# UT-Austin-RPL/GIGA

Measured on AMD Instinct MI355X. Metric: scenes/sec, higher is better.
Workload: dtype f32

## Files before the change

giga_amd/csrc/giga_encoder.hip:

```cpp
#include <atomic>
#include <cstdlib>

#include "../../include/giga_hip.h"
#include "giga_dev.h"
#include "giga_conv16.h"
#include "giga_conv32.h"
#include "giga_wino.h"
#include "giga_bwd_mega.h"
#include "giga_args.h"

namespace giga {



constexpr int CV_RS = 44;
constexpr int CV_OFF = 3;
constexpr int CV_ROWS = 12;
constexpr int ci_red_units(int nw) { return nw == 4 ? 25 : 13; }
constexpr size_t ci_lds_bytes(int xw, int nw, bool f16class = false) {
    const size_t stage = ((size_t)(xw + 3) * (f16class ? CI16_SLAB : CV_ROWS * CV_RS) + 4) * sizeof(float);
    const size_t red = (size_t)nw * ci_red_units(nw) * 64 * 16;
    return stage > red ? stage : red;
}

#ifdef GIGA_TRACE
static __device__ long long g_ci_trace[8 * 64];
#define CI_T(idx) do { if (blockIdx.x == 43 && lane == 0) \
        g_ci_trace[wave * 64 + (idx)] = __builtin_amdgcn_s_memtime(); } while (0)
#else
#define CI_T(idx) do {} while (0)
#endif
template <typename TOut, int SXW, bool SPLIT = false, int NW = 8, bool LO = true, bool MASK = false>
__global__ __launch_bounds__(512) void convin_project_kernel(
    const float* __restrict__ tsdf,
    const float* __restrict__ wpk,
    const float* __restrict__ bias,
    TOut* __restrict__ planes,
    float* __restrict__ xz_partial,
    float* __restrict__ yz_partial,
    int B, uint4* __restrict__ relu_mask = nullptr) {
    constexpr int XW = NW * SXW, NT = NW * 64;
    constexpr bool F16C = SPLIT || sizeof(TOut) == 2;
    constexpr int RS = SPLIT ? CI16_RS : CV_RS, SLAB = SPLIT ? CI16_SLAB : CV_ROWS * CV_RS;
    extern __shared__ __attribute__((aligned(16))) float lds[];
    const int tid = threadIdx.x, lane = tid & 63;
    const int wave = __builtin_amdgcn_readfirstlane(tid >> 6);
    const int j = lane & 15, g = lane >> 4;
    int xp = blockIdx.x, wy = blockIdx.y, b = blockIdx.z;
    if constexpr (XW == RES) {
        const int i = blockIdx.x, nfull = (B >> 3) << 6;
        xp = 0;
        if (i < nfull) { const int xcd = i & 7, slot = i >> 3; b = (slot >> 3) * 8 + xcd; wy = slot & 7; }
        else           { b = i >> 3; wy = i & 7; }
    }
    const int grp = wy >> 1, chh = wy & 1;
    const int x0 = xp * XW;
    const float* vol = tsdf + (size_t)b * RES * RES * RES;
    CI_T(0);

    constexpr int SPP = NT / 120, NPASS = (XW + 2 + SPP - 1) / SPP;
    const int st_slab = tid / 120, st_e = tid - 120 * st_slab, st_yl = st_e / 10, st_q = st_e - 10 * st_yl;
    const int st_iy = 10 * grp - 1 + st_yl;
    const bool st_on = st_slab < SPP && st_iy >= 0 && st_iy < RES;
    const float* st_src = vol + ((size_t)(x0 - 1 + st_slab) * RES + st_iy) * RES + 4 * st_q;
    float4 vals[NPASS];
#pragma unroll
    for (int p = 0; p < NPASS; ++p) {
        const int xl = st_slab + SPP * p, ix = x0 - 1 + xl;
        vals[p] = make_float4(0.f, 0.f, 0.f, 0.f);
        if (st_on && xl < XW + 2 && ix >= 0 && ix < RES)
            vals[p] = *reinterpret_cast<const float4*>(st_src + (size_t)SPP * p * RES * RES);
    }
    CI_T(50);
    float wreg[7];
    half8 wsh = {0, 0, 0, 0, 0, 0, 0, 0}, wsl = wsh;
    if constexpr (SPLIT) {
        const half8* wsp = reinterpret_cast<const half8*>(wpk);
        wsh = wsp[(2 * chh) * 64 + lane];
        wsl = wsp[(2 * chh + 1) * 64 + lane];
    } else {
#pragma unroll
        for (int s = 0; s < 7; ++s) wreg[s] = wpk[(chh * 7 + s) * 64 + lane];
    }
    const int ch = 16 * chh + j;
    const float bn = bias[ch];
    int abase[7];
#pragma unroll
    for (int s = 0; s < 7; ++s) {
        int t = 4 * s + g;
        t = t > 26 ? 26 : t;
        abase[s] = (t / 9) * SLAB + ((j >> 3) + (t / 3) % 3) * RS + CV_OFF + 4 * ((j >> 2) & 1) + (j & 3) + t % 3;
    }
    int sbase[8];
#pragma unroll
    for (int e = 0; e < 8; ++e) {
        const int t = g == 0 ? ci16_read(0, e) : g == 1 ? ci16_read(1, e) : g == 2 ? ci16_read(2, e) : ci16_read(3, e);
        sbase[e] = (t / 9) * SLAB + ((j >> 3) + (t / 3) % 3) * RS + CV_OFF + 4 * ((j >> 2) & 1) + (j & 3) + t % 3;
    }
    f32x4v acc_yz[5][5];
#pragma unroll
    for (int ip = 0; ip < 5; ++ip)
#pragma unroll
        for (int zg = 0; zg < 5; ++zg) acc_yz[ip][zg] = f32x4v{0.f, 0.f, 0.f, 0.f};
    const float inv = 1.0f / RES;
    const size_t img_stride = (size_t)RES * RES * CD;
    TOut* plane_xy = planes + ((size_t)1 * B + b) * img_stride;
    TOut* plane_yz = planes + ((size_t)2 * B + b) * img_stride;
    float* xzp = xz_partial + ((size_t)grp * B + b) * img_stride;
    const f32x4v bias4 = {bn, bn, bn, bn};
    const f32x4v zero4 = {0.f, 0.f, 0.f, 0.f};
    const unsigned xz_lane_b = ((4 * (g & 1) + 2 * (g >> 1)) * RES * CD + ch) * 4u;
    auto xz_store = [&](const f32x4v& part, float* dst) {
        float a02 = part[0], b02 = part[2], a13 = part[1], b13 = part[3];
        lane32_swap(a02, b02);
        lane32_swap(a13, b13);
        store_f32_saddr(dst, xz_lane_b, a02 + b02);
        store_f32_saddr(dst + RES * CD, xz_lane_b, a13 + b13);
    };
    auto xy_store = [&](const f32x2v (&sz)[5], TOut* dst) {
#pragma unroll
        for (int ia = 0; ia < 5; ia += 2) {
            const int ib = ia + 1 < 5 ? ia + 1 : ia;
            float sa = sz[ia][0] + sz[ia][1], sb = sz[ib][0] + sz[ib][1];
            lane16_swap(sa, sb);
            if (ia != ib || (g & 1) == 0) {
                const int iy = grp * 10 + 2 * (ia + (g & 1) * (ib - ia)) + (g >> 1);
                dst[iy * RES * CD + ch] = (TOut)((sa + sb) * inv);
            }
        }
    };
    if (st_slab < SPP) {
        float* st_dst = lds + st_slab * SLAB + st_yl * RS + CV_OFF + 1 + 4 * st_q;
#pragma unroll
        for (int p = 0; p < NPASS; ++p) {
            if (st_slab + SPP * p >= XW + 2) break;
            float* dst = st_dst + SPP * p * SLAB;
            float4 val = vals[p];
            if constexpr (SPLIT) {
                float* v4 = reinterpret_cast<float*>(&val);
#pragma unroll
// ... 167 lines not shown
            const int u = u0 + ul, ip = u / 5, zg = u % 5, lg = ln >> 4, lj = ln & 15;
            const int iy = grp * 10 + 2 * ip + (lg >> 1), iz0 = 8 * zg + 4 * (lg & 1);
            const int di = (iz0 * RES + iy) * CD + 16 * chh + lj;
            if constexpr (XW == RES) {
#pragma unroll
                for (int r = 0; r < 4; ++r) plane_yz[di + r * RES * CD] = (TOut)(sum[r] * inv);
            } else {
#pragma unroll
                for (int r = 0; r < 4; ++r) yzp[di + r * RES * CD] = sum[r];
            }
        }
        CI_T(41 + rd);
    }
    CI_T(63);
}

template <typename TOut>
__global__ void plane_finalize_kernel(const float* __restrict__ xz_partial, const float* __restrict__ yz_partial,
                                      TOut* __restrict__ planes, int B, int nxp, unsigned* __restrict__ sync_words, int nsync) {
    const size_t per4 = (size_t)B * RES * RES * CD / 4;
    const size_t t = (size_t)blockIdx.x * blockDim.x + threadIdx.x;
    if (blockIdx.x == 0 && sync_words) for (int i = threadIdx.x; i < nsync; i += blockDim.x) sync_words[i] = 0u;
    if (t >= per4) return;
    const f32x4v* xs = reinterpret_cast<const f32x4v*>(xz_partial) + t;
    const f32x4v* ys = reinterpret_cast<const f32x4v*>(yz_partial) + t;
    typedef TOut out4 __attribute__((ext_vector_type(4)));
    f32x4v sx = (xs[0] + xs[per4]) + (xs[2 * per4] + xs[3 * per4]);
    out4 ox;
#pragma unroll
    for (int r = 0; r < 4; ++r) ox[r] = (TOut)(sx[r] * (1.0f / RES));
    *reinterpret_cast<out4*>(planes + 4 * t) = ox;
    if (nxp > 1) {
        f32x4v sy = ys[0];
        for (int k = 1; k < nxp; ++k) sy += ys[(size_t)k * per4];
        out4 oy;
#pragma unroll
        for (int r = 0; r < 4; ++r) oy[r] = (TOut)(sy[r] * (1.0f / RES));
        *reinterpret_cast<out4*>(planes + 2 * 4 * per4 + 4 * t) = oy;
    }
}

int enc_nxp(int B) { return B >= 32 ? 1 : 5; }

EncWs enc_workspace(int B, int precision) {
    const size_t es = precision == 1 ? 2 : 4;
    const size_t n = 3 * (size_t)B;
    EncWs w{};
    size_t at = 0;
    auto take = [&](size_t elems, size_t esz) { size_t o = at; at += align_up(elems * esz, 256); return o; };
    w.P0 = take(n * 1600 * 32, es); w.A0 = take(n * 1600 * 32, es); w.S0 = take(n * 1600 * 32, es);
    w.Q0 = take(n * 400 * 32, es);  w.A1 = take(n * 400 * 64, es);  w.S1 = take(n * 400 * 64, es);
    w.Q1 = take(n * 100 * 64, es);  w.A2 = take(n * 100 * 128, es); w.S2 = take(n * 100 * 128, es);
    w.U0 = take(n * 400 * 64, es);  w.A3 = take(n * 400 * 64, es);  w.A4 = take(n * 400 * 64, es);
    w.U1 = take(n * 1600 * 32, es); w.A5 = take(n * 1600 * 32, es); w.A6 = take(n * 1600 * 32, es);
    w.YZ = take((size_t)(4 + enc_nxp(B)) * B * 1600 * 32, 4);
    w.XZ = w.YZ;
    w.SYNC = take(MEGA_SYNC_WORDS * 4, 4);
    w.MASK = take((size_t)B * 8 * RES * 64 * 4, 4);
    w.total = at;
    return w;
}


#define GIGA_UNET_LAYERS(X)                              \
    X(0, CONV3, 32, 0, 32, 40, 40, 2, false, 2)          \
    X(1, CONV3, 32, 0, 32, 40, 40, 2, true, 2)           \
    X(2, CONV3, 32, 0, 64, 20, 20, 1, false, 4)          \
    X(3, CONV3, 64, 0, 64, 20, 20, 1, true, 4)           \
    X(4, CONV3, 64, 0, 128, 10, 10, 1, false, 4)         \
    X(5, CONV3, 128, 0, 128, 10, 10, 1, false, 2)        \
    X(6, UPCONV, 128, 0, 64, 10, 10, 2, false, 2)        \
    X(7, CONV3, 64, 64, 64, 20, 20, 1, false, 2)         \
    X(8, CONV3, 64, 0, 64, 20, 20, 1, false, 4)          \
    X(9, UPCONV, 64, 0, 32, 20, 20, 2, false, 2)         \
    X(10, CONV3, 32, 32, 32, 40, 40, 2, false, 2)        \
    X(11, CONV3, 32, 0, 32, 40, 40, 2, false, 2)         \
    X(12, CONV1, 32, 0, 32, 40, 40, 2, false, 2)

struct MegaArgs {
    ConvArgs layer[NCONV];
    unsigned* sync;
    int nlayers;
    unsigned wino_mask;
};
constexpr int MEGA_GROUP = 8;
constexpr int MEGA_SLOTS = 4;
constexpr int MEGA_GROUP_MAX_IMG = 32;
constexpr int MEGA_NW = CONV_NW;
constexpr unsigned long long MEGA_SPIN_TICKS = 20ull * 100000000ull;
constexpr int MEGA_MAX_IN_FLIGHT = 4;

template <typename T, int MATH, bool WINO = false>
constexpr size_t mega_lds_bytes() {
    size_t m = 0;
#define X(l, KIND, C0, C1, COUT, H, W, NB, POOL, NB16) \
    { constexpr size_t v = conv_lds_bytes<T, KIND, C0, C1, COUT, H, W, (sizeof(T) == 2 ? NB16 : NB), MATH, (WINO ? WINO_NW : CONV_NW)>(); m = v > m ? v : m; \
      if constexpr (WINO && KIND == CONV3) { constexpr size_t u = wino_lds_bytes<C0, C1, H, W>(); m = u > m ? u : m; } }
    GIGA_UNET_LAYERS(X)
#undef X
    return m;
}

#ifdef GIGA_TRACE
static __device__ long long g_mega_trace[8][32];
#endif
__device__ __forceinline__ void xcd_barrier(unsigned* counter, unsigned target, int idx, int trace_row) {
#ifdef GIGA_TRACE
    if (threadIdx.x == 0 && trace_row >= 0 && trace_row < 8 && idx < 16) g_mega_trace[trace_row][2 * idx] = __builtin_amdgcn_s_memtime();
#endif
    if (threadIdx.x == 0) {
        __hip_atomic_fetch_add(counter, 1u, __ATOMIC_RELAXED, __HIP_MEMORY_SCOPE_WORKGROUP);
        unsigned spins = 0;
        unsigned long long t0 = 0;
        while (__hip_atomic_load(counter, __ATOMIC_RELAXED, __HIP_MEMORY_SCOPE_AGENT) < target) {
            __builtin_amdgcn_s_sleep(1);
            if ((++spins & 1023u) == 0) {
                const unsigned long long now = __builtin_amdgcn_s_memrealtime();
                if (t0 == 0) t0 = now;
                else if (now - t0 > MEGA_SPIN_TICKS) __builtin_trap();
            }
        }
    }
    __syncthreads();
#ifdef GIGA_TRACE
    if (threadIdx.x == 0 && trace_row >= 0 && trace_row < 8 && idx < 16) g_mega_trace[trace_row][2 * idx + 1] = __builtin_amdgcn_s_memtime();
#endif
}

__device__ __forceinline__ void xcd_arrive(unsigned* counter) {
    if (threadIdx.x == 0) __hip_atomic_fetch_add(counter, 1u, __ATOMIC_RELAXED, __HIP_MEMORY_SCOPE_WORKGROUP);
}
__device__ __forceinline__ void xcd_wait(unsigned* counter, unsigned target) {
    if (threadIdx.x == 0) {
        unsigned spins = 0;
        unsigned long long t0 = 0;
        while (__hip_atomic_load(counter, __ATOMIC_RELAXED, __HIP_MEMORY_SCOPE_AGENT) < target) {
            __builtin_amdgcn_s_sleep(1);
            if ((++spins & 1023u) == 0) {
                const unsigned long long now = __builtin_amdgcn_s_memrealtime();
                if (t0 == 0) t0 = now;
                else if (now - t0 > MEGA_SPIN_TICKS) __builtin_trap();
            }
        }
    }
    __syncthreads();
}

template <typename T, int KIND, int C0, int C1, int COUT, int H, int W>
__device__ __forceinline__ ConvArgs conv_image_range(ConvArgs a, int img0, int n) {
    constexpr int IH = KIND == DOWN ? 2 * H : H, IW = KIND == DOWN ? 2 * W : W;
    constexpr int OH = KIND == UPCONV ? 2 * H : H, OW = KIND == UPCONV ? 2 * W : W;
    const size_t s0 = (size_t)IH * IW * (a.cs0 ? a.cs0 : C0), s1 = (size_t)IH * IW * (a.cs1 ? a.cs1 : C1);
    a.in0 = reinterpret_cast<const T*>(a.in0) + img0 * s0;
    if (a.in1) a.in1 = reinterpret_cast<const T*>(a.in1) + img0 * s1;
    a.out = reinterpret_cast<T*>(a.out) + (size_t)img0 * OH * OW * COUT;
    if (a.out_pool) a.out_pool = reinterpret_cast<T*>(a.out_pool) + (size_t)img0 * (H / 2) * (W / 2) * COUT;
    if (a.out_nchw) a.out_nchw += (size_t)img0 * COUT * H * W;
    if (a.mask) a.mask += (size_t)img0 * OH * OW * COUT;
    a.nimg = n;
    if (img0 != 0) a.trace_id = -2;
    return a;
}

template <typename T, int MATH, bool WINO = false>
__global__ __launch_bounds__((WINO ? WINO_NW : MEGA_NW) * 64) void unet_mega_kernel(MegaArgs m) {
    extern __shared__ __attribute__((aligned(16))) uint8_t smem[];
    __shared__ unsigned s_place[2];
    if (threadIdx.x == 0) {
        const unsigned xcc = (unsigned)(__builtin_amdgcn_s_getreg((4 - 1) << 11 | 0 << 6 | 20) & 7);
        s_place[0] = xcc;
        s_place[1] = __hip_atomic_fetch_add(m.sync + xcc * 32, 1u, __ATOMIC_RELAXED, __HIP_MEMORY_SCOPE_WORKGROUP);
    }
    __syncthreads();
    const int xcd = (int)s_place[0], ticket = (int)s_place[1];
    const int nq = (int)gridDim.x >> 3, slot = ticket / MEGA_GROUP, q = slot * 8 + xcd, nimg = m.layer[0].nimg;
    if (slot >= nq >> 3) return;
    const int img0 = (q * nimg + nq - 1) / nq, per = ((q + 1) * nimg + nq - 1) / nq - img0;
    if (per == 0) return;
    const int block = ticket - slot * MEGA_GROUP, nblocks = MEGA_GROUP;
    unsigned* counter = m.sync + (8 + q) * 32;
    unsigned epoch = 0;
    auto is_wino = [&](auto kind_tag, int l) { return WINO && decltype(kind_tag)::value == CONV3 && (m.wino_mask >> l & 1u); };
#define X(l, KIND, C0, C1, COUT, H, W, NB, POOL, NB16)                                                                     \
    if (l < m.nlayers) {                                                                                                   \
        const ConvArgs a = conv_image_range<T, KIND, C0, C1, COUT, H, W>(m.layer[l], img0, per);                           \
        bool direct = true;                                                                                                \
        if constexpr (WINO && KIND == CONV3) {                                                                             \
            if (is_wino(std::integral_constant<int, KIND>{}, l)) {                                                         \
                direct = false;                                                                                            \
                _Pragma("unroll") for (int k = 0; k < wino_kpass(C0 + C1); ++k) {                                          \
                    if (l == 0 || k > 0) wino_fill<C0, C1, COUT>(a, smem, block, nblocks, k);                              \
                    wino_run<C0, C1, COUT, H, W, POOL, true>(a, smem, block, nblocks, k);                                  \
                    __builtin_amdgcn_s_waitcnt(0x0F70);                                                                    \
                    __syncthreads();                                                                                       \
                }                                                                                                          \
            }                                                                                                              \
        }                                                                                                                  \
        if constexpr (WINO && KIND == UPCONV) {                                                                            \
            if (m.wino_mask >> l & 1u) {                                                                                   \
                direct = false;                                                                                            \
                up_run<C0, COUT, H, W>(a, smem, block, nblocks);                                                           \
                __builtin_amdgcn_s_waitcnt(0x0F70);                                                                        \
                __syncthreads();                                                                                           \
            }                                                                                                              \
        }                                                                                                                  \
        if (direct) {                                                                                                      \
        if (l == 0) conv16_fill<T, KIND, C0, C1, COUT, (sizeof(T) == 2 ? NB16 : NB), MATH>(a, smem, block, nblocks);                \
        conv16_run<T, KIND, C0, C1, COUT, H, W, (sizeof(T) == 2 ? NB16 : NB), POOL, KIND == CONV3, MATH, (WINO ? WINO_NW : CONV_NW)>(a, smem, block, nblocks); \
        __builtin_amdgcn_s_waitcnt(0x0F70);                          \
        __syncthreads();                                      \
        }                                                                                                                  \
    }
#define NEXT(l, KIND, C0, C1, COUT, H, W, NB, POOL, NB16)                                                                  \
    if (l < m.nlayers) {                                                                                                   \
        bool direct = true;                                                                                                \
        if constexpr (WINO && KIND == CONV3) {                                                                             \
            if (is_wino(std::integral_constant<int, KIND>{}, l)) { direct = false; wino_fill<C0, C1, COUT>(m.layer[l], smem, block, nblocks, 0); } \
        }                                                                                                                  \
        if constexpr (WINO && KIND == UPCONV) {                                                                            \
            if (m.wino_mask >> l & 1u) { direct = false; up_fill<C0, COUT>(m.layer[l], smem, block, nblocks); }            \
        }                                                                                                                  \
        if (direct) conv16_fill<T, KIND, C0, C1, COUT, (sizeof(T) == 2 ? NB16 : NB), MATH>(m.layer[l], smem, block, nblocks);       \
        xcd_barrier(counter, ++epoch * (unsigned)nblocks, l, img0 == 0 ? block : -1);                                                                 \
    }
    X(0, CONV3, 32, 0, 32, 40, 40, 2, false, 2)
    NEXT(1, CONV3, 32, 0, 32, 40, 40, 2, true, 2)
    X(1, CONV3, 32, 0, 32, 40, 40, 2, true, 2)
    NEXT(2, CONV3, 32, 0, 64, 20, 20, 1, false, 4)
    X(2, CONV3, 32, 0, 64, 20, 20, 1, false, 4)
    NEXT(3, CONV3, 64, 0, 64, 20, 20, 1, true, 4)
    X(3, CONV3, 64, 0, 64, 20, 20, 1, true, 4)
    NEXT(4, CONV3, 64, 0, 128, 10, 10, 1, false, 4)
    X(4, CONV3, 64, 0, 128, 10, 10, 1, false, 4)
    NEXT(5, CONV3, 128, 0, 128, 10, 10, 1, false, 2)
    X(5, CONV3, 128, 0, 128, 10, 10, 1, false, 2)
    NEXT(6, UPCONV, 128, 0, 64, 10, 10, 2, false, 2)
    X(6, UPCONV, 128, 0, 64, 10, 10, 2, false, 2)
    NEXT(7, CONV3, 64, 64, 64, 20, 20, 1, false, 2)
    X(7, CONV3, 64, 64, 64, 20, 20, 1, false, 2)
    NEXT(8, CONV3, 64, 0, 64, 20, 20, 1, false, 4)
    X(8, CONV3, 64, 0, 64, 20, 20, 1, false, 4)
    NEXT(9, UPCONV, 64, 0, 32, 20, 20, 2, false, 2)
    X(9, UPCONV, 64, 0, 32, 20, 20, 2, false, 2)
    NEXT(10, CONV3, 32, 32, 32, 40, 40, 2, false, 2)
    X(10, CONV3, 32, 32, 32, 40, 40, 2, false, 2)
    NEXT(11, CONV3, 32, 0, 32, 40, 40, 2, false, 2)
    X(11, CONV3, 32, 0, 32, 40, 40, 2, false, 2)
    NEXT(12, CONV1, 32, 0, 32, 40, 40, 2, false, 2)
    X(12, CONV1, 32, 0, 32, 40, 40, 2, false, 2)
#undef NEXT
#undef X
}

#define GIGA_UNET_BWD_STAGES(X, P)                       \
    X(0, CONV1, 32, 0, 32, 40, 40, 2)                    \
    X(1, CONV3, 32, 0, 32, 40, 40, 2)                    \
    X(2, CONV3, 32, 0, 64, 40, 40, 2)                    \
    X(3, DOWN, 32, 0, 64, 20, 20, 2)                     \
    X(4, CONV3, 64, 0, 64, 20, 20, 1)                    \
    X(5, CONV3, 64, 0, 128, 20, 20, 1)                   \
    X(6, DOWN, 64, 0, 128, 10, 10, 1)                    \
    X(7, CONV3, 128, 0, 128, 10, 10, 1)                  \
    X(8, CONV3, 128, 0, 64, 10, 10, 1)                   \
    P(0)                                                 \
    X(9, CONV3, 64, 0, 64, 20, 20, 1)                    \
    X(10, CONV3, 64, 0, 32, 20, 20, 2)                   \
    P(1)                                                 \
    X(11, CONV3, 32, 0, 32, 40, 40, 2)                   \
    X(12, CONV3, 32, 0, 32, 40, 40, 2)
template <int MATH>
constexpr size_t bwd_mega_lds_bytes() {
    size_t m = 0;
#define X(k, KIND, C0, C1, COUT, H, W, NB) { constexpr size_t v = conv_lds_bytes<float, KIND, C0, C1, COUT, H, W, NB, MATH>(); m = v > m ? v : m; }
#define P(k)
    GIGA_UNET_BWD_STAGES(X, P)
#undef X
#undef P
    return m;
}
__device__ __forceinline__ void bwd_pool_stage(const BwdPool& p, int img0, int per, int block, int nblocks) {
    const int C4 = p.C >> 2;
    const unsigned total = (unsigned)per * p.H * p.W * C4;
    for (unsigned i = (unsigned)block * blockDim.x + threadIdx.x; i < total; i += (unsigned)nblocks * blockDim.x) {
        const int c = 4 * (int)(i % C4);
        const unsigned pl = i / C4;
        const int x = (int)(pl % p.W), y = (int)((pl / p.W) % p.H);
        const size_t img = (size_t)img0 + pl / ((unsigned)p.W * p.H);
        const size_t pix = (size_t)img0 * p.H * p.W + pl;
        const size_t qi = ((img * (p.H / 2) + y / 2) * (p.W / 2) + x / 2) * p.C + c;
        const float4 s4 = *reinterpret_cast<const float4*>(p.S + pix * p.C + c);
        const float4 d = *reinterpret_cast<const float4*>(p.dcat + pix * p.cs + p.coff + c);
        const float4 q = *reinterpret_cast<const float4*>(p.Q + qi);
        const float4 g = *reinterpret_cast<const float4*>(p.dQ + qi);
        float4 o;
        o.x = s4.x > 0.f ? d.x + (s4.x == q.x ? g.x : 0.f) : 0.f;
        o.y = s4.y > 0.f ? d.y + (s4.y == q.y ? g.y : 0.f) : 0.f;
        o.z = s4.z > 0.f ? d.z + (s4.z == q.z ? g.z : 0.f) : 0.f;
        o.w = s4.w > 0.f ? d.w + (s4.w == q.w ? g.w : 0.f) : 0.f;
        *reinterpret_cast<float4*>(p.dS + pix * p.C + c) = o;
    }
}
template <int MATH>
__global__ __launch_bounds__(MEGA_NW * 64) void unet_dgrad_mega_kernel(BwdMegaArgs m) {
    extern __shared__ __attribute__((aligned(16))) uint8_t smem[];
    __shared__ unsigned s_place[2];
    if (threadIdx.x == 0) {
// ... 132 lines not shown
    for (int i = 0; i < MegaSlots::MEGA_TRACKED; ++i) {
        if ((m.used[i] || m.pending[i]) && m.stream[i] == s) { mine = i; continue; }
        if (m.used[i] && !m.pending[i] && hipEventQuery(m.ev[i]) == hipSuccess) m.used[i] = false;
        if (m.used[i] || m.pending[i]) ++others;
        else if (spare < 0) spare = i;
    }
    int slot = mine >= 0 ? mine : spare;
    if (others >= MEGA_MAX_IN_FLIGHT || slot < 0) slot = -1;
    else if (!m.ev[slot] && hipEventCreateWithFlags(&m.ev[slot], hipEventDisableTiming) != hipSuccess) slot = -1;
    if (slot >= 0) { m.pending[slot] = true; m.stream[slot] = s; }
    m.busy.clear(std::memory_order_release);
    return slot;
}
static void persistent_launched(int slot, hipStream_t s) {
    if (slot < 0) return;
    int dev = 0;
    if (hipGetDevice(&dev) != hipSuccess || dev < 0 || dev >= 16) return;
    MegaSlots& m = g_mega_slots[dev];
    while (m.busy.test_and_set(std::memory_order_acquire)) {}
    if (hipEventRecord(m.ev[slot], s) == hipSuccess) { m.used[slot] = true; m.stream[slot] = s; }
    m.pending[slot] = false;
    m.busy.clear(std::memory_order_release);
}

void persistent_forget() {
    for (MegaSlots& m : g_mega_slots) {
        while (m.busy.test_and_set(std::memory_order_acquire)) {}
        for (int i = 0; i < MegaSlots::MEGA_TRACKED; ++i) { m.used[i] = false; m.pending[i] = false; m.ev[i] = nullptr; m.stream[i] = nullptr; }
        m.busy.clear(std::memory_order_release);
    }
}

int launch_unet_dgrad_mega(BwdMegaArgs m, bool bf16, hipStream_t s) {
    static const int env_persist = [] { const char* e = getenv("GIGA_UNET_PERSIST"); return e ? atoi(e) : -1; }();
    const int nimg = m.layer[0].nimg;
    int dev = 0, cus = 0;
    if (hipGetDevice(&dev) != hipSuccess || hipDeviceGetAttribute(&cus, hipDeviceAttributeMultiprocessorCount, dev) != hipSuccess) return 0;
    if (cus != 256 || env_persist == 0 || (env_persist < 0 && nimg < 24)) return 0;
    const int slot = persistent_slot(s);
    if (slot == -1) return 0;
    for (int k = 0; k < 13; ++k) m.layer[k].xcd_local = 0;
    if (hipMemsetAsync(m.sync, 0, MEGA_SYNC_WORDS * sizeof(unsigned), s) != hipSuccess) { persistent_launched(slot, s); return -10; }
    const int slots = (nimg + 7) / 8 < MEGA_SLOTS ? (nimg + 7) / 8 : MEGA_SLOTS;
    const unsigned grid = 8u * (unsigned)slots * MEGA_GROUP;
    if (bf16) {
        constexpr size_t lds = bwd_mega_lds_bytes<MATH_BF16>();
        static_assert(lds <= 160 * 1024, "LDS budget of the persistent data-gradient kernel");
        auto kern = unet_dgrad_mega_kernel<MATH_BF16>;
        giga::dyn_lds_once(reinterpret_cast<const void*>(kern), (int)lds);
        GIGA_LAUNCH(kern, dim3(grid), dim3(MEGA_NW * 64), lds, s, m);
    } else {
        constexpr size_t lds = bwd_mega_lds_bytes<MATH_NATIVE>();
        static_assert(lds <= 160 * 1024, "LDS budget of the persistent data-gradient kernel");
        auto kern = unet_dgrad_mega_kernel<MATH_NATIVE>;
        giga::dyn_lds_once(reinterpret_cast<const void*>(kern), (int)lds);
        GIGA_LAUNCH(kern, dim3(grid), dim3(MEGA_NW * 64), lds, s, m);
    }
    persistent_launched(slot, s);
    return hipGetLastError() == hipSuccess ? 1 : -10;
}

struct Probe { int stage; hipEvent_t ev0, ev1; };

static std::atomic<int> g_last_unet_path{0};

template <typename T, int MATH = MATH_NATIVE>
static int encoder_run(const float* tsdf, const uint8_t* blob, void* planes_nhwc, float* planes_nchw, int B,
                       uint8_t* ws, hipStream_t s, const Probe& pr, bool fold_final, int persist, int conv32, bool keep_mask = false,
                       unsigned wino_req = 0) {
    constexpr bool SPLIT = MATH == MATH_SPLIT;
    int stage_no = 0;
    auto pre = [&]() { if (pr.stage == stage_no) (void)hipEventRecord(pr.ev0, s); };
    auto post = [&]() { if (pr.stage == stage_no) (void)hipEventRecord(pr.ev1, s); ++stage_no; };
    constexpr int precision = sizeof(T) == 2 ? 1 : 0;
    const PackOff ko = pack_offsets();
    const EncWs w = enc_workspace(B, precision);
    T* P0 = reinterpret_cast<T*>(ws + w.P0);
    const size_t per = (size_t)B * RES * RES * CD;
    float* XZP = reinterpret_cast<float*>(ws + w.YZ);
    float* YZP = XZP + 4 * per;
    const int nxp = enc_nxp(B);
    static const int bf_ci16 = [] { const char* e = getenv("GIGA_BF16_CONVIN"); return e ? atoi(e) : 2; }();
    uint4* mask_out = keep_mask ? reinterpret_cast<uint4*>(ws + w.MASK) : nullptr;
    auto run_convin = [&](auto f16c, auto lo, auto msk) {
        constexpr bool CI_F16 = decltype(f16c)::value, CI_LO = decltype(lo)::value, MK = decltype(msk)::value;
        const float* cw = reinterpret_cast<const float*>(blob + (CI_F16 ? ko.convin_ws : ko.convin_w));
        const float* cb = reinterpret_cast<const float*>(blob + ko.convin_b);
        constexpr int NW = 8;
        if (nxp == 1) {
            auto kern = convin_project_kernel<T, RES / NW, CI_F16, NW, CI_LO, MK>;
            constexpr size_t lds = ci_lds_bytes(RES, NW, CI_F16);
            giga::dyn_lds_once(reinterpret_cast<const void*>(kern), (int)lds);
            GIGA_LAUNCH(kern, dim3(8 * B), dim3(NW * 64), lds, s, tsdf, cw, cb, P0, XZP, YZP, B, mask_out);
        } else {
            auto kern = convin_project_kernel<T, 8 / NW, CI_F16, NW, CI_LO, MK>;
            constexpr size_t lds = ci_lds_bytes(8, NW, CI_F16);
            giga::dyn_lds_once(reinterpret_cast<const void*>(kern), (int)lds);
            GIGA_LAUNCH(kern, dim3(5, 8, B), dim3(NW * 64), lds, s, tsdf, cw, cb, P0, XZP, YZP, B, mask_out);
        }
    };
    pre();
    using TT = std::true_type; using FF = std::false_type;
    if constexpr (SPLIT) run_convin(TT{}, TT{}, FF{});
    else if constexpr (sizeof(T) == 2) run_convin(TT{}, FF{}, FF{});
    else if constexpr (MATH == MATH_BF16) {
        if (bf_ci16 == 2 && keep_mask) run_convin(TT{}, FF{}, TT{});
        else if (bf_ci16) { if (keep_mask) run_convin(TT{}, TT{}, TT{}); else run_convin(TT{}, TT{}, FF{}); }
        else { if (keep_mask) run_convin(FF{}, FF{}, TT{}); else run_convin(FF{}, FF{}, FF{}); }
    } else { if (keep_mask) run_convin(FF{}, FF{}, TT{}); else run_convin(FF{}, FF{}, FF{}); }
    post();
    {
        pre();
        GIGA_LAUNCH(plane_finalize_kernel<T>, dim3((unsigned)((per / 4 + 255) / 256)), dim3(256), 0, s, XZP, YZP, P0, B,
                           nxp, reinterpret_cast<unsigned*>(ws + w.SYNC), MEGA_SYNC_WORDS);
        post();
    }
    if (hipGetLastError() != hipSuccess) return -10;

    const int nimg = 3 * B;
    const int xcd_local = [] { const char* e = getenv("GIGA_CONV_XCD"); return e ? atoi(e) : 1; }();
    constexpr bool CAN_WINO = sizeof(T) == 4 && MATH == MATH_NATIVE;
    unsigned wino_mask = 0;
    if constexpr (CAN_WINO) {
        for (int l = 0; l < NCONV; ++l)
            if ((kConv[l].kind == CONV3 || kConv[l].kind == UPCONV) && (wino_req >> l & 1u)) wino_mask |= 1u << l;
    }
    auto W_ = [&](int l) {
        if ((wino_mask >> l & 1u) && kConv[l].kind == CONV3) return blob + ko.conv[l].wino;
        return blob + (SPLIT ? ko.conv[l].w16s : MATH == MATH_BF16 ? ko.conv[l].wbf : precision == 1 ? ko.conv[l].w16 : ko.conv[l].w32);
    };
    auto Bi = [&](int l) { return reinterpret_cast<const float*>(blob + ko.conv[l].bias); };
    auto args = [&](int l, const void* i0, const void* i1, void* o, void* op) {
        ConvArgs a{};
        a.in0 = i0; a.in1 = i1; a.w = W_(l); a.bias = Bi(l); a.out = o; a.out_pool = op; a.out_nchw = nullptr;
        a.nimg = nimg;
        a.trace_id = l;
        a.xcd_local = xcd_local;
        return a;
    };
    uint8_t* b = ws;
    int rc = 0;
    void* a6 = fold_final ? planes_nhwc : static_cast<void*>(b + w.A6);
    ConvArgs L[NCONV] = {
        args(0, b + w.P0, nullptr, b + w.A0, nullptr),  args(1, b + w.A0, nullptr, b + w.S0, b + w.Q0),
        args(2, b + w.Q0, nullptr, b + w.A1, nullptr),  args(3, b + w.A1, nullptr, b + w.S1, b + w.Q1),
        args(4, b + w.Q1, nullptr, b + w.A2, nullptr),  args(5, b + w.A2, nullptr, b + w.S2, nullptr),
        args(6, b + w.S2, nullptr, b + w.U0, nullptr),  args(7, b + w.U0, b + w.S1, b + w.A3, nullptr),
        args(8, b + w.A3, nullptr, b + w.A4, nullptr),  args(9, b + w.A4, nullptr, b + w.U1, nullptr),
        args(10, b + w.U1, b + w.S0, b + w.A5, nullptr), args(11, b + w.A5, nullptr, a6, nullptr),
        args(12, b + w.A6, nullptr, planes_nhwc, nullptr)};
    L[12].out_nchw = planes_nchw;
    const int nlayers = fold_final ? 12 : 13;
    static const int env_persist = [] { const char* e = getenv("GIGA_UNET_PERSIST"); return e ? atoi(e) : -1; }();
    const bool full_device = [] {
        int dev = 0, cus = 0;
        if (hipGetDevice(&dev) != hipSuccess) return false;
        if (hipDeviceGetAttribute(&cus, hipDeviceAttributeMultiprocessorCount, dev) != hipSuccess) return false;
        return cus == 256;
    }();
    constexpr bool F16CLASS = sizeof(T) == 2 || MATH == MATH_SPLIT;
    const bool probe_layer = pr.stage >= 2 && pr.stage <= 14;
    const bool by_default = F16CLASS || nimg >= 24;
    bool mega = full_device && !probe_layer &&
                (persist > 0 || (persist == 0 && (env_persist > 0 || (env_persist < 0 && by_default))));
    int mega_slot = -2;
    if (mega) { mega_slot = persistent_slot(s); mega = mega_slot != -1; }
    constexpr int C32MODE = sizeof(T) == 2 ? C32_NATIVE : MATH == MATH_SPLIT ? C32_SPLIT : MATH == MATH_BF16 ? C32_BF16 : -1;
    constexpr int C32_AUTO_MAX_IMAGES = 48;
    static const int env_c32 = [] { const char* e = getenv("GIGA_CONV32"); return e ? (atoi(e) ? 1 : -1) : 0; }();
    if constexpr (C32MODE >= 0) {
        const int want = conv32 != 0 ? conv32 : env_c32 != 0 ? env_c32 : (nimg <= C32_AUTO_MAX_IMAGES ? 1 : -1);
        if (want > 0) {
            auto W32 = [&](int l) { return blob + (C32MODE == C32_SPLIT ? ko.conv[l].c32s : C32MODE == C32_BF16 ? ko.conv[l].c32b : ko.conv[l].c32h); };
            ConvArgs M[NCONV];
            for (int l = 0; l < NCONV; ++l) { M[l] = L[l]; M[l].w = W32(l); M[l].xcd_local = 0; M[l].out_pool = nullptr; }
            M[2].in0 = b + w.S0; M[2].out_pool = b + w.Q0;
            M[4].in0 = b + w.S1; M[4].out_pool = b + w.Q1;
            if (mega) {
                MegaArgs m{};
                for (int l = 0; l < NCONV; ++l) m.layer[l] = M[l];
                m.sync = reinterpret_cast<unsigned*>(b + w.SYNC);
                m.nlayers = nlayers;
                const unsigned grid = (unsigned)c32_groups(nimg) * MEGA_GROUP;
                static const int env_fuse = [] { const char* e = getenv("GIGA_C32_FUSE"); return e ? atoi(e) : -1; }();
                const int groups = c32_groups(nimg);
                const bool fuse = env_fuse >= 0 ? env_fuse != 0 : (nimg + groups - 1) / groups <= 2;
                stage_no = 15;
                pre();
                auto go = [&](auto kern) {
                    giga::dyn_lds_once(reinterpret_cast<const void*>(kern), C32_LDS_TOTAL);
                    GIGA_LAUNCH(kern, dim3(grid), dim3(C32_NW * 64), C32_LDS_TOTAL, s, m);
                };
                if (fuse) go(unet32_mega_kernel<C32MODE, true>); else go(unet32_mega_kernel<C32MODE, false>);
                g_last_unet_path.store(GIGA_PATH_CONV32 | GIGA_PATH_PERSISTENT | (fuse ? GIGA_PATH_FUSED_PAIRS : 0), std::memory_order_relaxed);
                persistent_launched(mega_slot, s);
                post();
                return hipGetLastError() == hipSuccess ? 0 : -10;
            }
            g_last_unet_path.store(GIGA_PATH_CONV32, std::memory_order_relaxed);
            if (pr.stage == 15) (void)hipEventRecord(pr.ev0, s);
#define X(l, KIND, C0, C1, COUT, H, W, POOLIN, SPW, SGN, SGS, KPS)                                                          \
            if (l < nlayers) { pre(); rc |= launch_conv32<typename U32Layer<C32MODE, l>::G, U32Layer<C32MODE, l>::RELU>(M[l], s); post(); } \
            else { pre(); post(); }
            GIGA_UNET32_LAYERS(X)
#undef X
            if (pr.stage == 15) (void)hipEventRecord(pr.ev1, s);
            return rc;
        }
    }
    g_last_unet_path.store((mega ? GIGA_PATH_PERSISTENT : 0) | (wino_mask ? GIGA_PATH_WINOGRAD : 0), std::memory_order_relaxed);
    if (mega) {
        MegaArgs m{};
        for (int l = 0; l < NCONV; ++l) { m.layer[l] = L[l]; m.layer[l].xcd_local = 0; }
        m.sync = reinterpret_cast<unsigned*>(b + w.SYNC);
        m.nlayers = nlayers;
        m.wino_mask = wino_mask;
        const int slots = (nimg + 7) / 8 < MEGA_SLOTS ? (nimg + 7) / 8 : MEGA_SLOTS;
        const unsigned grid = 8u * (unsigned)slots * MEGA_GROUP;
        stage_no = 15;
        auto go = [&](auto kern, const size_t lds, const int nw) {
            giga::dyn_lds_once(reinterpret_cast<const void*>(kern), (int)lds);
            pre();
            GIGA_LAUNCH(kern, dim3(grid), dim3(nw * 64), lds, s, m);
            persistent_launched(mega_slot, s);
            post();
        };
        constexpr size_t lds = mega_lds_bytes<T, MATH>();
        static_assert(lds <= 160 * 1024, "LDS budget of the persistent U-Net kernel");
        if constexpr (CAN_WINO) {
            constexpr size_t ldsw = mega_lds_bytes<T, MATH, true>();
            static_assert(ldsw <= 160 * 1024, "LDS budget of the persistent U-Net kernel (Winograd stages)");
            if (wino_mask) go(unet_mega_kernel<T, MATH, true>, ldsw, WINO_NW); else go(unet_mega_kernel<T, MATH, false>, lds, MEGA_NW);
        } else {
            go(unet_mega_kernel<T, MATH, false>, lds, MEGA_NW);
        }
        return hipGetLastError() == hipSuccess ? 0 : -10;
    }
    if (pr.stage == 15) (void)hipEventRecord(pr.ev0, s);
#define X(l, KIND, C0, C1, COUT, H, W, NB, POOL, NB16)                                                                    \
    if (l < nlayers) {                                                                                                    \
        pre();                                                                                                            \
        bool direct = true;                                                                                               \
        if constexpr (CAN_WINO && KIND == CONV3) {                                                                        \
            if (wino_mask >> l & 1u) { direct = false; rc |= launch_wino<C0, C1, COUT, H, W, POOL>(L[l], s); }            \
        }                                                                                                                 \
        if constexpr (CAN_WINO && KIND == UPCONV) {                                                                       \
            if (wino_mask >> l & 1u) { direct = false; rc |= launch_up<C0, COUT, H, W>(L[l], s); }                        \
        }                                                                                                                 \
        if (direct) rc |= launch_conv<T, KIND, C0, C1, COUT, H, W, (sizeof(T) == 2 ? NB16 : NB), POOL, KIND == CONV3, MATH>(L[l], s); \
        post();                                                                                                           \
    }                                                                                                                     \
    else { pre(); post(); }
    GIGA_UNET_LAYERS(X)
#undef X
    if (pr.stage == 15) (void)hipEventRecord(pr.ev1, s);
    return rc;
}

int launch_encoder(const float* tsdf, const uint8_t* blob, void* planes_nhwc, float* planes_nchw, int B,
                   int precision, uint8_t* ws, hipStream_t s, int probe_stage, void* ev0, void* ev1) {
    if (B <= 0) return 0;
    Probe pr{ev0 && ev1 ? probe_stage : -1, static_cast<hipEvent_t>(ev0), static_cast<hipEvent_t>(ev1)};
    const bool fold = (precision & GIGA_FOLD_FINAL) != 0;
    const int persist = (precision & GIGA_LAYERWISE_UNET) ? -1 : (precision & GIGA_PERSIST_UNET) ? 1 : 0;
    const int prec = precision & ~(GIGA_FOLD_FINAL | GIGA_PERSIST_UNET | GIGA_LAYERWISE_UNET | GIGA_CONV32_UNET | GIGA_CONV16_UNET | GIGA_CONVIN_MASK | GIGA_DIRECT_CONV);
    const int c32 = (precision & GIGA_CONV32_UNET) ? 1 : (precision & GIGA_CONV16_UNET) ? -1 : 0;
    const bool km = (precision & GIGA_CONVIN_MASK) != 0;
    static const unsigned env_wino = [] { const char* e = getenv("GIGA_WINOGRAD"); return e ? (unsigned)strtoul(e, nullptr, 0) : WINO_DEFAULT_MASK; }();
    const unsigned wino = (precision & GIGA_DIRECT_CONV) ? 0u : env_wino;
    if (prec == 2) return encoder_run<float, MATH_SPLIT>(tsdf, blob, planes_nhwc, planes_nchw, B, ws, s, pr, fold, persist, c32);
    if (prec == 3) return encoder_run<float, MATH_BF16>(tsdf, blob, planes_nhwc, planes_nchw, B, ws, s, pr, fold, persist, c32, km);
    return prec == 1 ? encoder_run<half_t>(tsdf, blob, planes_nhwc, planes_nchw, B, ws, s, pr, fold, persist, c32)
                     : encoder_run<float>(tsdf, blob, planes_nhwc, planes_nchw, B, ws, s, pr, fold, persist, c32, km, wino);
}

}

extern "C" int giga_encoder_last_path(void) { return giga::g_last_unet_path.load(std::memory_order_relaxed); }

#ifdef GIGA_TRACE
extern "C" int giga_debug_mega_trace(long long* host_out) {
    return hipMemcpyFromSymbol(host_out, HIP_SYMBOL(giga::g_mega_trace), sizeof(long long) * 8 * 32) == hipSuccess ? 0 : -10;
}
extern "C" int giga_debug_c32_trace(long long* host_out) {
    return hipMemcpyFromSymbol(host_out, HIP_SYMBOL(giga::g_c32_trace), sizeof(long long) * giga::NCONV * giga::C32_NW * 8) == hipSuccess ? 0 : -10;
}
extern "C" int giga_debug_convin_trace(long long* host_out) {
    return hipMemcpyFromSymbol(host_out, HIP_SYMBOL(giga::g_ci_trace), sizeof(long long) * 8 * 64) == hipSuccess ? 0 : -10;
}
extern "C" int giga_debug_conv_trace(int layer, long long* host_out) {
    if (!host_out) {
        static const long long zeros[giga::CONV_NW * 64] = {};
        if (hipMemcpyToSymbol(HIP_SYMBOL(giga::g_conv_trace), zeros, sizeof(zeros)) != hipSuccess) return -10;
        return hipMemcpyToSymbol(HIP_SYMBOL(giga::g_conv_trace_layer), &layer, sizeof(int)) == hipSuccess ? 0 : -10;
    }
    return hipMemcpyFromSymbol(host_out, HIP_SYMBOL(giga::g_conv_trace), sizeof(long long) * giga::CONV_NW * 64) == hipSuccess ? 0 : -10;
}
#endif
```

Measured before the change: 94060.

## Fold plane finalize into persistent U-Net kernel and zero sync words in convin

When the persistent native-f32 U-Net path is used, the plane finalize step (summing partial xz/yz projections and scaling) runs inside the mega kernel for each group's own image range, instead of as a separate launch. Sync-word clearing moves into the first block of the convin kernel. Layer 0's fill is then issued early via NEXT so it is not redone. This removes one kernel launch and its dependency gap, and lets the first layer's fill follow the freshly written planes. The cost is more complexity in mega-kernel scheduling and a reliance on correct per-group image ranges.

```diff
diff --git a/giga_amd/csrc/giga_encoder.hip b/giga_amd/csrc/giga_encoder.hip
--- a/giga_amd/csrc/giga_encoder.hip
+++ b/giga_amd/csrc/giga_encoder.hip
@@ -38,7 +38,8 @@
     TOut* __restrict__ planes,
     float* __restrict__ xz_partial,
     float* __restrict__ yz_partial,
-    int B, uint4* __restrict__ relu_mask = nullptr) {
+    int B, uint4* __restrict__ relu_mask = nullptr,
+    unsigned* __restrict__ sync_words = nullptr) {
     constexpr int XW = NW * SXW, NT = NW * 64;
     constexpr bool F16C = SPLIT || sizeof(TOut) == 2;
     constexpr int RS = SPLIT ? CI16_RS : CV_RS, SLAB = SPLIT ? CI16_SLAB : CV_ROWS * CV_RS;
@@ -56,6 +57,8 @@
     const int grp = wy >> 1, chh = wy & 1;
     const int x0 = xp * XW;
     const float* vol = tsdf + (size_t)b * RES * RES * RES;
+    if (sync_words && blockIdx.x == 0 && blockIdx.y == 0 && blockIdx.z == 0)
+        for (int i = tid; i < MEGA_SYNC_WORDS; i += NT) sync_words[i] = 0u;
     CI_T(0);
 
     constexpr int SPP = NT / 120, NPASS = (XW + 2 + SPP - 1) / SPP;
@@ -389,6 +392,9 @@
     unsigned* sync;
     int nlayers;
     unsigned wino_mask;
+    const float* fin_xz;
+    const float* fin_yz;
+    int fin_nxp;
 };
 constexpr int MEGA_GROUP = 8;
 constexpr int MEGA_SLOTS = 4;
@@ -487,6 +493,7 @@
     const int block = ticket - slot * MEGA_GROUP, nblocks = MEGA_GROUP;
     unsigned* counter = m.sync + (8 + q) * 32;
     unsigned epoch = 0;
+    bool filled0 = false;
     auto is_wino = [&](auto kind_tag, int l) { return WINO && decltype(kind_tag)::value == CONV3 && (m.wino_mask >> l & 1u); };
 #define X(l, KIND, C0, C1, COUT, H, W, NB, POOL, NB16)                                                                     \
     if (l < m.nlayers) {                                                                                                   \
@@ -496,7 +503,7 @@
             if (is_wino(std::integral_constant<int, KIND>{}, l)) {                                                         \
                 direct = false;                                                                                            \
                 _Pragma("unroll") for (int k = 0; k < wino_kpass(C0 + C1); ++k) {                                          \
-                    if (l == 0 || k > 0) wino_fill<C0, C1, COUT>(a, smem, block, nblocks, k);                              \
+                    if ((l == 0 && !filled0) || k > 0) wino_fill<C0, C1, COUT>(a, smem, block, nblocks, k);                \
                     wino_run<C0, C1, COUT, H, W, POOL, true>(a, smem, block, nblocks, k);                                  \
                     __builtin_amdgcn_s_waitcnt(0x0F70);                                                                    \
                     __syncthreads();                                                                                       \
@@ -512,7 +519,7 @@
             }                                                                                                              \
         }                                                                                                                  \
         if (direct) {                                                                                                      \
-        if (l == 0) conv16_fill<T, KIND, C0, C1, COUT, (sizeof(T) == 2 ? NB16 : NB), MATH>(a, smem, block, nblocks);                \
+        if (l == 0 && !filled0) conv16_fill<T, KIND, C0, C1, COUT, (sizeof(T) == 2 ? NB16 : NB), MATH>(a, smem, block, nblocks);    \
         conv16_run<T, KIND, C0, C1, COUT, H, W, (sizeof(T) == 2 ? NB16 : NB), POOL, KIND == CONV3, MATH, (WINO ? WINO_NW : CONV_NW)>(a, smem, block, nblocks); \
         __builtin_amdgcn_s_waitcnt(0x0F70);                          \
         __syncthreads();                                      \
@@ -529,6 +536,34 @@
         }                                                                                                                  \
         if (direct) conv16_fill<T, KIND, C0, C1, COUT, (sizeof(T) == 2 ? NB16 : NB), MATH>(m.layer[l], smem, block, nblocks);       \
         xcd_barrier(counter, ++epoch * (unsigned)nblocks, l, img0 == 0 ? block : -1);                                                                 \
+    }
+    if constexpr (sizeof(T) == 4 && MATH == MATH_NATIVE) {
+        if (m.fin_xz) {
+            const int B = nimg / 3;
+            const int xlo = img0, xhi = img0 + per < B ? img0 + per : B;
+            const int ylo = img0 > 2 * B ? img0 : 2 * B, yhi = m.fin_nxp > 1 ? img0 + per : 0;
+            if (xlo < xhi || ylo < yhi) {
+                constexpr size_t Q = RES * RES * CD / 4;
+                const size_t per4 = (size_t)B * Q;
+                const f32x4v* xs = reinterpret_cast<const f32x4v*>(m.fin_xz);
+                const f32x4v* ys = reinterpret_cast<const f32x4v*>(m.fin_yz);
+                f32x4v* p0 = reinterpret_cast<f32x4v*>(const_cast<void*>(m.layer[0].in0));
+                const size_t me = (size_t)block * blockDim.x + threadIdx.x, stride = (size_t)nblocks * blockDim.x;
+                for (size_t t = xlo * Q + me; t < xhi * Q; t += stride) {
+                    const f32x4v sx = (xs[t] + xs[t + per4]) + (xs[t + 2 * per4] + xs[t + 3 * per4]);
+                    p0[t] = sx * (1.0f / RES);
+                }
+                for (size_t t = (ylo - 2 * B) * Q + me; ylo < yhi && t < (yhi - 2 * B) * Q; t += stride) {
+                    f32x4v sy = ys[t];
+                    for (int k = 1; k < m.fin_nxp; ++k) sy += ys[(size_t)k * per4 + t];
+                    p0[2 * per4 + t] = sy * (1.0f / RES);
+                }
+                __builtin_amdgcn_s_waitcnt(0x0F70);
+                __syncthreads();
+                filled0 = true;
+                NEXT(0, CONV3, 32, 0, 32, 40, 40, 2, false, 2)
+            }
+        }
     }
     X(0, CONV3, 32, 0, 32, 40, 40, 2, false, 2)
     NEXT(1, CONV3, 32, 0, 32, 40, 40, 2, true, 2)
@@ -827,6 +862,27 @@
     const int nxp = enc_nxp(B);
     static const int bf_ci16 = [] { const char* e = getenv("GIGA_BF16_CONVIN"); return e ? atoi(e) : 2; }();
     uint4* mask_out = keep_mask ? reinterpret_cast<uint4*>(ws + w.MASK) : nullptr;
+
+    const int nimg = 3 * B;
+    static const int env_persist = [] { const char* e = getenv("GIGA_UNET_PERSIST"); return e ? atoi(e) : -1; }();
+    const bool full_device = [] {
+        int dev = 0, cus = 0;
+        if (hipGetDevice(&dev) != hipSuccess) return false;
+        if (hipDeviceGetAttribute(&cus, hipDeviceAttributeMultiprocessorCount, dev) != hipSuccess) return false;
+        return cus == 256;
+    }();
+    constexpr bool F16CLASS = sizeof(T) == 2 || MATH == MATH_SPLIT;
+    const bool probe_layer = pr.stage >= 2 && pr.stage <= 14;
+    const bool by_default = F16CLASS || nimg >= 24;
+    bool mega = full_device && !probe_layer &&
+                (persist > 0 || (persist == 0 && (env_persist > 0 || (env_persist < 0 && by_default))));
+    const bool fold_fin = sizeof(T) == 4 && MATH == MATH_NATIVE && mega;
+    unsigned* const sync_words = reinterpret_cast<unsigned*>(ws + w.SYNC);
+    unsigned* const ci_sync = fold_fin ? sync_words : nullptr;
+    auto run_finalize = [&]() {
+        GIGA_LAUNCH(plane_finalize_kernel<T>, dim3((unsigned)((per / 4 + 255) / 256)), dim3(256), 0, s, XZP, YZP, P0, B,
+                    nxp, sync_words, MEGA_SYNC_WORDS);
+    };
     auto run_convin = [&](auto f16c, auto lo, auto msk) {
         constexpr bool CI_F16 = decltype(f16c)::value, CI_LO = decltype(lo)::value, MK = decltype(msk)::value;
         const float* cw = reinterpret_cast<const float*>(blob + (CI_F16 ? ko.convin_ws : ko.convin_w));
@@ -836,12 +892,12 @@
             auto kern = convin_project_kernel<T, RES / NW, CI_F16, NW, CI_LO, MK>;
             constexpr size_t lds = ci_lds_bytes(RES, NW, CI_F16);
             giga::dyn_lds_once(reinterpret_cast<const void*>(kern), (int)lds);
-            GIGA_LAUNCH(kern, dim3(8 * B), dim3(NW * 64), lds, s, tsdf, cw, cb, P0, XZP, YZP, B, mask_out);
+            GIGA_LAUNCH(kern, dim3(8 * B), dim3(NW * 64), lds, s, tsdf, cw, cb, P0, XZP, YZP, B, mask_out, ci_sync);
         } else {
             auto kern = convin_project_kernel<T, 8 / NW, CI_F16, NW, CI_LO, MK>;
             constexpr size_t lds = ci_lds_bytes(8, NW, CI_F16);
             giga::dyn_lds_once(reinterpret_cast<const void*>(kern), (int)lds);
-            GIGA_LAUNCH(kern, dim3(5, 8, B), dim3(NW * 64), lds, s, tsdf, cw, cb, P0, XZP, YZP, B, mask_out);
+            GIGA_LAUNCH(kern, dim3(5, 8, B), dim3(NW * 64), lds, s, tsdf, cw, cb, P0, XZP, YZP, B, mask_out, ci_sync);
         }
     };
     pre();
@@ -854,15 +910,11 @@
         else { if (keep_mask) run_convin(FF{}, FF{}, TT{}); else run_convin(FF{}, FF{}, FF{}); }
     } else { if (keep_mask) run_convin(FF{}, FF{}, TT{}); else run_convin(FF{}, FF{}, FF{}); }
     post();
-    {
-        pre();
-        GIGA_LAUNCH(plane_finalize_kernel<T>, dim3((unsigned)((per / 4 + 255) / 256)), dim3(256), 0, s, XZP, YZP, P0, B,
-                           nxp, reinterpret_cast<unsigned*>(ws + w.SYNC), MEGA_SYNC_WORDS);
-        post();
-    }
+    pre();
+    if (!fold_fin) run_finalize();
+    post();
     if (hipGetLastError() != hipSuccess) return -10;
 
-    const int nimg = 3 * B;
     const int xcd_local = [] { const char* e = getenv("GIGA_CONV_XCD"); return e ? atoi(e) : 1; }();
     constexpr bool CAN_WINO = sizeof(T) == 4 && MATH == MATH_NATIVE;
     unsigned wino_mask = 0;
@@ -896,20 +948,12 @@
         args(12, b + w.A6, nullptr, planes_nhwc, nullptr)};
     L[12].out_nchw = planes_nchw;
     const int nlayers = fold_final ? 12 : 13;
-    static const int env_persist = [] { const char* e = getenv("GIGA_UNET_PERSIST"); return e ? atoi(e) : -1; }();
-    const bool full_device = [] {
-        int dev = 0, cus = 0;
-        if (hipGetDevice(&dev) != hipSuccess) return false;
-        if (hipDeviceGetAttribute(&cus, hipDeviceAttributeMultiprocessorCount, dev) != hipSuccess) return false;
-        return cus == 256;
-    }();
-    constexpr bool F16CLASS = sizeof(T) == 2 || MATH == MATH_SPLIT;
-    const bool probe_layer = pr.stage >= 2 && pr.stage <= 14;
-    const bool by_default = F16CLASS || nimg >= 24;
-    bool mega = full_device && !probe_layer &&
-                (persist > 0 || (persist == 0 && (env_persist > 0 || (env_persist < 0 && by_default))));
     int mega_slot = -2;
     if (mega) { mega_slot = persistent_slot(s); mega = mega_slot != -1; }
+    if (fold_fin && !mega) {
+        run_finalize();
+        if (hipGetLastError() != hipSuccess) return -10;
+    }
     constexpr int C32MODE = sizeof(T) == 2 ? C32_NATIVE : MATH == MATH_SPLIT ? C32_SPLIT : MATH == MATH_BF16 ? C32_BF16 : -1;
     constexpr int C32_AUTO_MAX_IMAGES = 48;
     static const int env_c32 = [] { const char* e = getenv("GIGA_CONV32"); return e ? (atoi(e) ? 1 : -1) : 0; }();
@@ -960,6 +1004,7 @@
         m.sync = reinterpret_cast<unsigned*>(b + w.SYNC);
         m.nlayers = nlayers;
         m.wino_mask = wino_mask;
+        if (fold_fin) { m.fin_xz = XZP; m.fin_yz = YZP; m.fin_nxp = nxp; }
         const int slots = (nimg + 7) / 8 < MEGA_SLOTS ? (nimg + 7) / 8 : MEGA_SLOTS;
         const unsigned grid = 8u * (unsigned)slots * MEGA_GROUP;
         stage_no = 15;
```

New measurement: 95050, median of 6. 1.01x the previous value.
